# ska-telescope/ska-sdp-screen-fitting

Measured on AMD Instinct MI355X. Metric: screen-slots/sec (ant×time×freq) + FITS-cube wall-clock, KL 256² screen, higher is better.
Workload: dtype f64

## Files before the change

### include/screenfit.h

```cpp
#ifndef SCREENFIT_H
#define SCREENFIT_H

#include <stddef.h>
#include <stdint.h>

#ifdef __cplusplus
extern "C" {
#endif

#define SF_OK 0
#define SF_EINVAL (-22)
#define SF_ENOMEM (-12)
#define SF_EIO (-5)
#define SF_ENODEV (-19)

#define SF_MAX_DIR 60
#define SF_MAX_FIT_DIR 128
#define SF_MAX_EVAL_DIR 128

#define SF_SCREEN_PHASE 0
#define SF_SCREEN_TEC 1
#define SF_SCREEN_AMPLITUDE 2

#define SF_EVAL_NAN_SCRUB 1u
// ... 32 lines not shown
#define SF_OPT_EVAL_XCD_MAP 7
#define SF_OPT_EVAL_GROUPS 8
#define SF_OPT_EVAL_BANDS 9
#define SF_OPT_FIT_LEAN 10
#define SF_OPT_TESS_SLOTS 11
#define SF_OPT_TESS_WAVES 12
#define SF_OPT_TESS_TILE 13
#define SF_OPT_TESS_BOX 14
#define SF_OPT_EVAL_INT 15
#define SF_OPT_EVAL_WG_WAVES 16
#define SF_OPT_FIT_EIG_WAVES 17
#define SF_OPT_FIT_SUBSET_DELETION 18
#define SF_OPT_FIT_WIDE_CACHE 19
#define SF_OPT_FIT_WIDE_POOL_MB 20
#define SF_OPT_FIT_WIDE_POOL_MAX 21
#define SF_EVAL_KERNEL_AUTO 0
#define SF_EVAL_KERNEL_TILE 1
#define SF_EVAL_KERNEL_LDS4 2
#define SF_EVAL_KERNEL_LDS8 3
#define SF_EVAL_KERNEL_LDS16 4
#define SF_EVAL_KERNEL_LDS8H 5
#define SF_EVAL_KERNEL_LDS16H 6
#define SF_EVAL_KERNEL_TILE3 7
#define SF_EVAL_KERNEL_SHB 8
#define SF_EVAL_KERNEL_WIDE 9
int sf_get_eval_kernel(sf_ctx* ctx, int gain, unsigned flags, int* kernel);
#define SF_EVAL_CONTRACTION_F64 0
#define SF_EVAL_CONTRACTION_I8_DIGITS 1
int sf_get_eval_contraction(sf_ctx* ctx, int gain, unsigned flags, int* contraction);
int sf_set_option(sf_ctx* ctx, int option, int value);
// ... 6 lines not shown
                 double beta);
int sf_set_basis_wide(sf_ctx* ctx, const double* pp_host, int D, double r0,
                      double beta);
int sf_get_basis(sf_ctx* ctx, double* c_host, double* pinv_c_host,
                 double* u_host, double* eig_host);

int sf_set_piercepoints(sf_ctx* ctx, const double* pp_host, int D, double r0,
                        double beta);

int sf_kl_fit(sf_ctx* ctx, const double* phase, const float* weight, int T,
              int F, int A, const int* station_order_host,
              const sf_fit_params* params, double* coef, double* resid,
              float* w_out, int32_t* order_out);

int sf_get_fit_stats(sf_ctx* ctx, int* n_masks, int* n_general);

int sf_get_fit_pool(sf_ctx* ctx, uint64_t* masks_host, double* entries_host,
                    int max_masks, int* n_masks);
int sf_get_fit_pool_wide(sf_ctx* ctx, uint64_t* masks_host, double* entries_host,
                         int max_masks, int* n_masks);

int sf_set_grid(sf_ctx* ctx, const double* x_host, int nx,
                const double* y_host, int ny);

int sf_kl_eval(sf_ctx* ctx, const double* coef, int64_t S, float* out,
               int64_t ring_slots, unsigned flags);

int sf_kl_eval_gain(sf_ctx* ctx, const double* coef_phase,
                    const double* coef_xx, const double* coef_yy, int64_t S,
                    float* out, int64_t ring_slots, unsigned flags);
// ... 27 lines not shown
```

### ska-sdp-screen-fitting_amd/csrc/capi.hip

```cpp
#include <hip/hip_runtime.h>

#include <cmath>
#include <cstring>
#include <string>
#include <vector>

#include "sf_internal.h"

namespace sf {
static thread_local std::string g_last_error;
void set_error(const std::string& msg) { g_last_error = msg; }
}

using sf::set_error;

namespace {

int check_device(int device) {
  int n = 0;
  hipError_t e = hipGetDeviceCount(&n);
  if (e != hipSuccess || n == 0) {
    set_error("no HIP device available");
    return SF_ENODEV;
  }
// ... 104 lines not shown
  hipFree(ctx->d_pfrag);
  hipFree(ctx->d_cdig);
  hipFree(ctx->d_kdig);
  hipFree(ctx->d_kflag);
  if (ctx->kdig_read) (void)hipEventDestroy(ctx->kdig_read);
  hipFree(ctx->d_skip);
  hipFree(ctx->d_st_order);
  hipFree(ctx->d_keys);
  hipFree(ctx->d_ids);
  hipFree(ctx->d_pool_mask);
  hipFree(ctx->d_pool);
  hipFree(ctx->d_pool_status);
  hipFree(ctx->d_pos);
  hipFree(ctx->d_sigma);
  hipFree(ctx->d_class);
  hipFree(ctx->d_counters);
  hipFree(ctx->d_scratch);
  hipFree(ctx->d_wscratch);
  hipFree(ctx->d_oscratch);
  hipFree(ctx->d_gw);
  hipFree(ctx->d_smooth);
  hipFree(ctx->d_tess_tab);
  hipFree(ctx->d_trash);
  delete ctx;
  return SF_OK;
}

int sf_set_stream(sf_ctx* ctx, void* stream) {
  SF_REQUIRE(ctx, SF_EINVAL, "sf_set_stream: NULL context");
  ctx->stream = reinterpret_cast<hipStream_t>(stream);
// ... 43 lines not shown
  SF_REQUIRE(ctx, SF_EINVAL, "sf_set_option: NULL context");
  switch (option) {
    case SF_OPT_FIT_GENERAL:
      ctx->force_general = value != 0;
      return SF_OK;
    case SF_OPT_EVAL_KERNEL:
      SF_REQUIRE(value >= SF_EVAL_KERNEL_AUTO && value <= SF_EVAL_KERNEL_WIDE,
                 SF_EINVAL, "sf_set_option: unknown evaluation kernel");
      ctx->eval_kernel = value;
      return SF_OK;
    case SF_OPT_FIT_PACK:
      ctx->fit_pack = value != 0;
      return SF_OK;
    case SF_OPT_FIT_LEAN:
      ctx->fit_lean = value != 0;
      return SF_OK;
    case SF_OPT_EVAL_KS_PAD:
      SF_REQUIRE(value >= 0 && value <= 3, SF_EINVAL,
                 "sf_set_option: k-step padding must be 0..3");
      ctx->eval_ks_pad = value;
      return SF_OK;
    case SF_OPT_EVAL_SLEEP:
      SF_REQUIRE(value >= 0 && value <= 1000, SF_EINVAL,
                 "sf_set_option: eval sleep must be 0..1000");
      ctx->eval_sleep = value;
      return SF_OK;
    case SF_OPT_EVAL_XCD_MAP:
      SF_REQUIRE(value >= -1 && value <= 1, SF_EINVAL,
                 "sf_set_option: XCD map must be -1, 0 or 1");
      ctx->eval_xcd_map = value;
// ... 272 lines not shown
                        order_out);
}

int sf_get_fit_stats(sf_ctx* ctx, int* n_masks, int* n_general) {
  SF_REQUIRE(ctx, SF_EINVAL, "sf_get_fit_stats: NULL context");
  int c[4] = {0, 0, 0, 0};
  SF_HIP(hipSetDevice(ctx->device));
  SF_HIP(hipStreamSynchronize(ctx->stream));
  if (ctx->d_counters)
    SF_HIP(hipMemcpy(c, ctx->d_counters, sizeof(c), hipMemcpyDeviceToHost));
  if (n_masks) *n_masks = c[0];
  if (n_general) *n_general = c[2];
  return SF_OK;
}

int sf_get_fit_pool(sf_ctx* ctx, uint64_t* masks_host, double* entries_host,
                    int max_masks, int* n_masks) {
  SF_REQUIRE(ctx && n_masks && max_masks >= 0, SF_EINVAL, "sf_get_fit_pool: bad argument");
  SF_REQUIRE(max_masks == 0 || (masks_host && entries_host), SF_EINVAL,
             "sf_get_fit_pool: NULL output");
  SF_REQUIRE(!ctx->wide, SF_EINVAL,
             "sf_get_fit_pool: 64-bit mask keys; above SF_MAX_DIR directions "
             "(sf_set_basis_wide) call sf_get_fit_pool_wide");
  SF_HIP(hipSetDevice(ctx->device));
  SF_HIP(hipStreamSynchronize(ctx->stream));
  int c0 = 0;
  if (ctx->d_counters)
    SF_HIP(hipMemcpy(&c0, ctx->d_counters, sizeof(int), hipMemcpyDeviceToHost));
  const int n = ctx->pool_D == ctx->D && (size_t)c0 <= ctx->pool_cap ? c0 : 0;
  *n_masks = n;
// ... 315 lines not shown
```

### ska-sdp-screen-fitting_amd/csrc/kl_fit_fast.hip

```cpp
#include <hip/hip_runtime.h>

#include <algorithm>
#include <cmath>
#include <cstdlib>

#include "kl_fit_steps.h"
#include "sf_internal.h"

namespace sf {

constexpr size_t kLdsBytes = 160 * 1024;
constexpr double kTinyW = kPinvAtol * 1.001;
constexpr unsigned long long kEmptyKey = 0ull;

__device__ __forceinline__ unsigned long long mix64(unsigned long long x) {
  x ^= x >> 30;
  x *= 0xbf58476d1ce4e5b9ull;
  x ^= x >> 27;
  x *= 0x94d049bb133111ebull;
  x ^= x >> 31;
  return x;
}

__device__ int table_insert(unsigned long long* keys, int cap,
// ... 7 lines not shown
  }
  return -3;
}

__device__ int table_find(const unsigned long long* keys, int cap,
                          unsigned long long key) {
  int h = (int)(mix64(key) & (unsigned long long)(cap - 1));
  for (int probe = 0; probe < cap; ++probe) {
    const unsigned long long k = keys[h];
    if (k == key) return h;
    if (k == kEmptyKey) return -1;
    h = (h + 1) & (cap - 1);
  }
  return -1;
}

template <int GW>
__global__ __launch_bounds__(256) void kl_classify_kernel(
    const float* __restrict__ weight, int64_t S, int F, int A, int D,
    const int* __restrict__ st_order, const uint8_t* __restrict__ skip,
    int ref_skip, unsigned long long* __restrict__ keys, int cap,
    int* __restrict__ pos, uint8_t* __restrict__ cls,
    int* __restrict__ counters,
    double* __restrict__ coef, double* __restrict__ resid,
    float* __restrict__ w_out, int32_t* __restrict__ order_out) {
  constexpr int kPerWave = 64 / GW;
  const int l = lane();
  const int g = l / GW;
  const int d = l % GW;
  const int64_t s = ((int64_t)blockIdx.x * (blockDim.x / 64) + threadIdx.x / 64) *
// ... 599 lines not shown
    v0[l] = fabs(lm) > kPinvAtol ? sh / lm : 0.0;
  }
  lds_sync();
  double wa = 0.0;
  if (l < D)
#pragma unroll kMatVecUnroll
    for (int r = 0; r < D; ++r) wa += L.U[l * ld + r] * v0[r];
  lds_sync();
  white_d = wa;
  resid_d = phi_d - model_value<M>(screen_type, sall);
}

#ifndef SF_FIT_MINW
#define SF_FIT_MINW 4
#endif
template <bool SLOW, int SPW, bool LEAN>
__global__ __launch_bounds__(256, SLOW ? 1 : SF_FIT_MINW) void kl_fit_pass_kernel(
    int it, int niter, int64_t S, int F, int A, int D,
    const double* __restrict__ phase, const double* __restrict__ refph,
    int ref_sub, const double* __restrict__ g_u, const double* __restrict__ g_c,
    const double* __restrict__ g_eig, const int* __restrict__ st_order,
    const uint8_t* __restrict__ cls, int* __restrict__ pos,
    const int* __restrict__ ids, unsigned long long* __restrict__ keys, int cap,
    const double* __restrict__ pool, int pool_cap, int* __restrict__ counters,
    int screen_type, double nsigma, int adjust_order, double* __restrict__ coef,
    double* __restrict__ resid, float* __restrict__ w_out,
    int32_t* __restrict__ order_out) {
#pragma clang fp contract(off)
  extern __shared__ double smem[];
  const int ld = odd_ld(D);
  using G = Group<SPW>;
  using M = FitMath<!SLOW>;
  const G tm;
  constexpr bool CG = SPW == 1;
  const int nwaves = blockDim.x / 64;
  const int nslots = nwaves * SPW;
  const int wv = (threadIdx.x / 64) * SPW + G::index();
  const int d = G::lane();
  double* sU = smem;
  double* sC = CG ? nullptr : sU + D * ld;
  double* sl = sU + (CG ? 1 : 2) * D * ld;
  for (int e = threadIdx.x; e < D * D; e += blockDim.x) {
    const int r = e / D, c = e % D;
// ... 15 lines not shown
    L.pr = nullptr;
  } else {
    L.Vs = wb;
    L.G = wb + D * ld;
    L.M = L.G + D * ld;
    L.lams = (SLOW ? L.M + D * ld : L.G + D * ld);
    L.vec = L.lams + 64;
    L.cs = reinterpret_cast<double2*>(L.vec + 6 * 64);
    L.pr = reinterpret_cast<int2*>(L.cs + 64);
  }
  const uint8_t want = SLOW ? 2 : 0;

  for (int64_t s = (int64_t)blockIdx.x * nslots + wv; s < S;
       s += (int64_t)gridDim.x * nslots) {
    if (SLOW && cls[s] != want) continue;
    const uint8_t cl = SLOW ? want : cls[s];
    const int a = (int)(s % A);
    const int p0 = pos[s];
    const int64_t base = s * D;
    double phi_d = 0.0, w_d = 0.0, white_d = 0.0, resid_d = 0.0;
    if (d < D) {
      phi_d = phase_ref(phase, refph, ref_sub, s, a, A, D, d);
      w_d = (double)w_out[base + d];
      white_d = it == 0 ? 0.0 : coef[base + d];
      resid_d = it == 0 ? 0.0 : resid[base + d];
    }
    double order = (double)order_out[s];
    const double station_order = (double)st_order[a];
    if (cl != want) continue;
    int id = -1;
    if (p0 >= 0) {
      id = ids[p0];
      if (id < 0 || id >= pool_cap) {
        if (d == 0) atomicOr(counters + 3, 1);
        continue;
      }
    } else if (p0 == -3) {
      if (d == 0) atomicOr(counters + 3, 2);
      continue;
    }
    const bool unfl = (d < D) && (w_d > 0.0);
    const unsigned long long um = G::ballot(unfl);
    const int n_unfl = __popcll(um);

// ... 249 lines not shown
                       ctx->stream, ctx->d_c, D, ctx->d_pool_mask, (int)ctx->pool_cap, \
                       ctx->d_counters, ctx->d_pool, done);                            \
  } while (0)
    switch (nw) {
      case 1: SF_LAUNCH_EIG(1); break;
      case 2: SF_LAUNCH_EIG(2); break;
      case 4: SF_LAUNCH_EIG(4); break;
      default: SF_LAUNCH_EIG(3); break;
    }
#undef SF_LAUNCH_EIG
    SF_HIP(hipGetLastError());
  }
  return SF_OK;
}

template <bool SLOW, int SPW, bool LEAN>
static int launch_pass_spw(sf_ctx* ctx, int it, const sf_fit_params* p,
                           const RefSpec& r, int64_t S, int F, int A,
                           const double* phase, double* coef, double* resid,
                           float* w_out, int32_t* order_out) {
  const int D = ctx->D;
  const size_t shared = fast_shared_bytes(D, SPW == 1);
  const size_t slot = fast_wave_bytes(D, SLOW, LEAN);
  int nw = 1, best = 0;
  for (int k = 1; k <= 4; ++k) {
    const size_t per_wg = shared + (size_t)k * SPW * slot;
    if (per_wg > kLdsBytes) break;
    const int waves = k * (int)(kLdsBytes / per_wg);
    if (waves > best) {
      best = waves;
      nw = k;
    }
  }
  const size_t shm = shared + (size_t)nw * SPW * slot;
  if (shm > 64 * 1024)
    SF_HIP(hipFuncSetAttribute(
        reinterpret_cast<const void*>(&kl_fit_pass_kernel<SLOW, SPW, LEAN>),
        hipFuncAttributeMaxDynamicSharedMemorySize, (int)shm));
  int64_t blocks = (S + nw * SPW - 1) / (nw * SPW);
  if (blocks > 16384) blocks = 16384;
  hipLaunchKernelGGL((kl_fit_pass_kernel<SLOW, SPW, LEAN>), dim3((unsigned)blocks),
                     dim3(64 * nw), shm, ctx->stream, it, p->niter, S, F, A, D,
                     phase, r.refph, r.sub, ctx->d_u, ctx->d_c, ctx->d_eig,
                     ctx->d_st_order, ctx->d_class, ctx->d_pos, ctx->d_ids,
                     ctx->d_keys, (int)ctx->table_cap, ctx->d_pool,
                     (int)ctx->pool_cap, ctx->d_counters, p->screen_type,
                     p->nsigma, p->adjust_order, coef, resid, w_out, order_out);
  SF_HIP(hipGetLastError());
  return SF_OK;
}

template <bool SLOW>
static int launch_pass(sf_ctx* ctx, int it, const sf_fit_params* p,
                       const RefSpec& r, int64_t S, int F, int A,
                       const double* phase, double* coef, double* resid,
                       float* w_out, int32_t* order_out, bool lean) {
  const bool pack = !SLOW && ctx->D <= 32 && ctx->fit_pack;
  if (!SLOW && lean && ctx->fit_lean) {
    if (pack)
      return launch_pass_spw<false, 2, true>(ctx, it, p, r, S, F, A, phase, coef,
                                             resid, w_out, order_out);
    return launch_pass_spw<false, 1, true>(ctx, it, p, r, S, F, A, phase, coef,
                                           resid, w_out, order_out);
  }
  if (pack)
    return launch_pass_spw<SLOW, 2, false>(ctx, it, p, r, S, F, A, phase, coef,
                                           resid, w_out, order_out);
  return launch_pass_spw<SLOW, 1, false>(ctx, it, p, r, S, F, A, phase, coef, resid,
                                         w_out, order_out);
}

int launch_block_sigma(sf_ctx* ctx, int T, int F, int A, const double* phase,
                       const RefSpec& r, int screen_type, const double* resid,
                       const float* w_out) {
  hipLaunchKernelGGL(kl_block_sigma_kernel, dim3(F * A), dim3(256), 0,
                     ctx->stream, T, F, A, ctx->D, phase, r.refph, r.sub,
                     ctx->d_skip, r.skip, screen_type, resid, w_out,
                     ctx->d_sigma);
  SF_HIP(hipGetLastError());
  return SF_OK;
}

int fit_buffers(sf_ctx* ctx, int64_t S, int F, int A, double** resid,
                float** w_out, int32_t** order_out) {
// ... 6 lines not shown
    SF_TRY_RC(grow(&ctx->d_wscratch, ctx->wscratch_cap, n));
    *w_out = ctx->d_wscratch;
  }
  if (!*order_out) {
    SF_TRY_RC(grow(&ctx->d_oscratch, ctx->oscratch_cap, (size_t)S));
    *order_out = ctx->d_oscratch;
  }
  SF_TRY_RC(grow(&ctx->d_sigma, ctx->sigma_cap, (size_t)F * A));
  SF_TRY_RC(grow(&ctx->d_counters, ctx->counters_cap, 8));
  return SF_OK;
}

int launch_fit(sf_ctx* ctx, const double* phase, const float* weight, int T,
               int F, int A, const sf_fit_params* p, double* coef,
               double* resid, float* w_out, int32_t* order_out) {
  if (ctx->wide)
    return launch_fit_wide(ctx, phase, weight, T, F, A, p, coef, resid, w_out,
                           order_out);
  const int D = ctx->D;
  const int64_t S = (int64_t)T * F * A;
  const RefSpec r = ref_spec(p, A);
  SF_TRY_RC(launch_skip(ctx, phase, weight, T, F, A, r));

  static const char* env = std::getenv("SCREENFIT_FIT");
  if (ctx->force_general || (env && env[0] == 'g')) {
    if (p->screen_type == SF_SCREEN_AMPLITUDE ||
        (p->niter > 1 && p->screen_type != SF_SCREEN_PHASE)) {
      set_error("the general fit kernel handles phase (any niter) and tec (niter 1) only");
      return SF_EINVAL;
    }
// ... 37 lines not shown
  hipLaunchKernelGGL(kl_classify_kernel<W>, grid, dim3(256), 0, ctx->stream,    \
                     weight, S, F, A, D, ctx->d_st_order, ctx->d_skip, r.skip,  \
                     ctx->d_keys, cap, ctx->d_pos, ctx->d_class,               \
                     ctx->d_counters, coef, resid, w_out, order_out)
    switch (gw) {
      case 8: SF_CLASSIFY(8); break;
      case 16: SF_CLASSIFY(16); break;
      case 32: SF_CLASSIFY(32); break;
      default: SF_CLASSIFY(64); break;
    }
#undef SF_CLASSIFY
    SF_HIP(hipGetLastError());
  }

  const bool block_flags = p->screen_type != SF_SCREEN_PHASE;
  for (int it = 0; it < p->niter; ++it) {
    int n_slow = 0, n_nonuniform = 0;
    SF_TRY_RC(number_and_decompose(ctx, &n_slow, &n_nonuniform));
    SF_TRY_RC(launch_pass<false>(ctx, it, p, r, S, F, A, phase, coef, resid,
                               w_out, order_out, n_nonuniform == 0));
    if (n_slow > 0)
      SF_TRY_RC(launch_pass<true>(ctx, it, p, r, S, F, A, phase, coef, resid,
                                w_out, order_out, false));
    if (block_flags && it + 1 < p->niter) {
      SF_TRY_RC(launch_block_sigma(ctx, T, F, A, phase, r, p->screen_type, resid,
                                 w_out));
      hipLaunchKernelGGL(kl_block_flag_kernel, dim3((unsigned)((S + 255) / 256)),
                         dim3(256), 0, ctx->stream, S, F, A, D, phase, r.refph,
                         r.sub, ctx->d_class, p->screen_type, p->nsigma,
                         ctx->d_sigma, resid, w_out, ctx->d_keys, cap,
                         ctx->d_pos);
      SF_HIP(hipGetLastError());
    }
  }
  int err = 0;
  SF_HIP(hipMemcpyAsync(&err, ctx->d_counters + 3, sizeof(int),
                        hipMemcpyDeviceToHost, ctx->stream));
  SF_HIP(hipStreamSynchronize(ctx->stream));
  SF_REQUIRE((err & 3) == 0, SF_EIO, "sf_kl_fit: internal mask table overflow");
  SF_REQUIRE((err & 4) == 0, SF_EIO,
             "sf_kl_fit: lean fit pass saw non-uniform weights in a slot "
             "classified uniform (slot left unwritten)");
  SF_REQUIRE((err & 8) == 0, SF_EIO,
             "sf_kl_fit: a mask with every direction unflagged entered the "
             "subset-basis pool (its basis is the global one; left unbuilt)");
  return SF_OK;
}

}
```

### ska-sdp-screen-fitting_amd/csrc/kl_fit_steps.h

```cpp
#pragma once

#include <hip/hip_runtime.h>

#include <cmath>

#include "screenfit.h"
#include "sf_wave.h"

namespace sf {

constexpr double kPinvAtol = 1e-3;
constexpr int kJacobiMaxSweeps = 40;

__host__ __device__ inline int odd_ld(int n) { return n | 1; }

inline __device__ __noinline__ void nl_sincos(double x, double* s, double* c) { sincos(x, s, c); }
inline __device__ __noinline__ double nl_atan2(double y, double x) { return atan2(y, x); }
inline __device__ __noinline__ double nl_log10(double x) { return log10(x); }
inline __device__ __noinline__ double nl_pow(double x, double y) { return pow(x, y); }
inline __device__ __noinline__ double nl_log(double x) { return log(x); }
inline __device__ __noinline__ double nl_fmod(double x, double y) { return fmod(x, y); }

template <bool NI>
struct FitMath {
// ... 11 lines not shown
  }
  static __device__ __forceinline__ double ln(double x) {
    if constexpr (NI) return nl_log(x); else return log(x);
  }
  static __device__ __forceinline__ double mod(double x, double y) {
    if constexpr (NI) return nl_fmod(x, y); else return fmod(x, y);
  }
};

__device__ __forceinline__ double phase_ref(const double* phase,
                                            const double* refph, int sub,
                                            int64_t s, int a, int A, int D,
                                            int d) {
  double v = phase[s * D + d];
  if (refph) v -= refph[(s / A) * D + d];
  else if (sub >= 0) v -= phase[(s + (sub - a)) * D + d];
  return v;
}

template <class Math = FitMath<false>>
__device__ __forceinline__ double model_value(int screen_type, double x) {
  return screen_type == SF_SCREEN_AMPLITUDE ? Math::power(10.0, x) : x;
}

template <class Math = FitMath<false>>
__device__ __forceinline__ double screen_diff(int screen_type, double val,
                                              double resid) {
  if (screen_type == SF_SCREEN_AMPLITUDE)
    return Math::lg10(val) - Math::lg10(fabs(val - resid));
  return resid;
// ... 151 lines not shown
```

### ska-sdp-screen-fitting_amd/csrc/sf_internal.h

```cpp
#pragma once

#include <hip/hip_runtime.h>

#include <cstdint>
#include <string>

#include "screenfit.h"

namespace sf {

void set_error(const std::string& msg);

#define SF_HIP(call)                                                        \
  do {                                                                      \
    hipError_t e_ = (call);                                                 \
    if (e_ != hipSuccess) {                                                 \
      ::sf::set_error(std::string(#call) + ": " + hipGetErrorString(e_));   \
      return SF_EIO;                                                        \
    }                                                                       \
  } while (0)

#define SF_REQUIRE(cond, code, msg) \
  do {                              \
    if (!(cond)) {                  \
// ... 125 lines not shown
  size_t tess_tab_cap = 0;
  int force_general = 0;
  int eval_kernel = SF_EVAL_KERNEL_AUTO;
  int64_t eval_max_blocks = 0;
  int eval_ks_pad = 0;
  int eval_sleep = 0;
  int eval_xcd_map = -1;
  int eval_groups = 0;
  int eval_bands = 0;
  int tess_slots = 0;
  int tess_waves = 0;
  int tess_tile = 0;
  int tess_box = -1;
  int fit_pack = 1;
  int fit_lean = 1;
};

namespace sf {
constexpr int kEvalMaxKS = 15;
constexpr int kEvalWideMaxKS = SF_MAX_EVAL_DIR / 4;
inline bool eval_int_applies(const sf_ctx* ctx, bool gain, unsigned flags,
                             bool out_aligned16) {
  return !gain && ctx->dig_ok && ctx->d_cdig && ctx->eval_int != 0 &&
         (flags & SF_EVAL_FAST_SINCOS) && ctx->n_pix % 4 == 0 && out_aligned16 &&
         ctx->ksteps >= 12 && ctx->ksteps <= kEvalMaxKS;
}

struct RefSpec {
  int sub = -1;
  const double* refph = nullptr;
// ... 56 lines not shown
```

### ska-sdp-screen-fitting_amd/ska_sdp_screen_fitting_amd/_lib.py

```python

import contextlib
import ctypes
import os
import threading

import numpy as np

_HERE = os.path.dirname(os.path.abspath(__file__))
LIB_PATH = os.environ.get("SCREENFIT_LIB", os.path.join(_HERE, "libscreenfit.so"))

SF_SCREEN_PHASE = 0
SF_SCREEN_TEC = 1
SF_SCREEN_AMPLITUDE = 2
SF_EVAL_NAN_SCRUB = 1
SF_EVAL_FAST_SINCOS = 1 << 8
SF_EVAL_NT_STORES = 1 << 9
SF_EVAL_BIG_ENDIAN = 1 << 10
SF_MAX_DIR = 60
SF_MAX_FIT_DIR = 128
SF_MAX_EVAL_DIR = 128
SF_MAX_POINTS = 4096
SF_OPT_FIT_GENERAL = 1
SF_OPT_EVAL_KERNEL = 2
SF_OPT_EVAL_MAX_BLOCKS = 3
# ... 3 lines not shown
SF_OPT_EVAL_XCD_MAP = 7
SF_OPT_EVAL_GROUPS = 8
SF_OPT_EVAL_BANDS = 9
SF_OPT_FIT_LEAN = 10
SF_OPT_TESS_SLOTS = 11
SF_OPT_TESS_WAVES = 12
SF_OPT_TESS_TILE = 13
SF_OPT_TESS_BOX = 14
SF_OPT_EVAL_INT = 15
SF_OPT_EVAL_WG_WAVES = 16
SF_OPT_FIT_EIG_WAVES = 17
SF_OPT_FIT_SUBSET_DELETION = 18
SF_OPT_FIT_WIDE_CACHE = 19
SF_OPT_FIT_WIDE_POOL_MB = 20
SF_OPT_FIT_WIDE_POOL_MAX = 21
SF_EVAL_KERNEL_AUTO = 0
SF_EVAL_KERNEL_TILE = 1
SF_EVAL_KERNEL_LDS4 = 2
SF_EVAL_KERNEL_LDS8 = 3
SF_EVAL_KERNEL_LDS16 = 4
SF_EVAL_KERNEL_LDS8H = 5
SF_EVAL_KERNEL_LDS16H = 6
SF_EVAL_KERNEL_TILE3 = 7
SF_EVAL_KERNEL_SHB = 8
SF_EVAL_KERNEL_WIDE = 9
EVAL_KERNEL_NAMES = {SF_EVAL_KERNEL_TILE: "kl_eval_kernel",
                     SF_EVAL_KERNEL_LDS4: "kl_eval_lds_kernel<4 waves>",
                     SF_EVAL_KERNEL_LDS8: "kl_eval_lds_kernel<8 waves>",
                     SF_EVAL_KERNEL_LDS16: "kl_eval_lds_kernel<16 waves>",
                     SF_EVAL_KERNEL_LDS8H: "kl_eval_lds_kernel<8 waves, 2 tiles>",
                     SF_EVAL_KERNEL_LDS16H: "kl_eval_lds_kernel<16 waves, 2 tiles>",
                     SF_EVAL_KERNEL_TILE3: "kl_eval_kernel<3 waves/SIMD>",
                     SF_EVAL_KERNEL_SHB: "kl_eval_kernel<Cpix in LDS>",
                     SF_EVAL_KERNEL_WIDE: "kl_eval_wide_kernel"}

EXPORTED = (
    "sf_version", "sf_last_error", "sf_create", "sf_destroy", "sf_set_stream",
    "sf_synchronize", "sf_set_option", "sf_get_eval_kernel", "sf_get_eval_contraction", "sf_alloc", "sf_free", "sf_copy_h2d", "sf_copy_d2h",
    "sf_set_basis", "sf_set_basis_wide", "sf_set_piercepoints", "sf_get_basis", "sf_kl_fit", "sf_get_fit_stats", "sf_get_fit_pool",
    "sf_get_fit_pool_wide",
    "sf_stream_create", "sf_stream_destroy", "sf_device_cus",
    "sf_set_grid", "sf_kl_eval", "sf_kl_eval_gain", "sf_kl_eval_sums",
    "sf_tess_fill", "sf_smooth",
    "sf_set_points", "sf_kl_eval_points", "sf_kl_eval_point_values",
    "sf_kl_eval_values",
)


_identity = {}


def library_identity(path=None):
    import hashlib
    p = os.path.realpath(path or LIB_PATH)
# ... 45 lines not shown
            "sf_synchronize": ([vp], c_int),
            "sf_set_option": ([vp, c_int, c_int], c_int),
            "sf_get_eval_kernel": ([vp, c_int, ctypes.c_uint, ip], c_int),
            "sf_get_eval_contraction": ([vp, c_int, ctypes.c_uint, ip], c_int),
            "sf_alloc": ([vp, ctypes.c_size_t, ctypes.POINTER(vp)], c_int),
            "sf_free": ([vp, vp], c_int),
            "sf_copy_h2d": ([vp, vp, vp, ctypes.c_size_t], c_int),
            "sf_copy_d2h": ([vp, vp, vp, ctypes.c_size_t], c_int),
            "sf_set_basis": ([vp, vp, c_int, c_dbl, c_dbl], c_int),
            "sf_set_basis_wide": ([vp, vp, c_int, c_dbl, c_dbl], c_int),
            "sf_set_piercepoints": ([vp, vp, c_int, c_dbl, c_dbl], c_int),
            "sf_get_basis": ([vp, vp, vp, vp, vp], c_int),
            "sf_kl_fit": ([vp, vp, vp, c_int, c_int, c_int, ip,
                           ctypes.POINTER(FitParams), vp, vp, vp, vp], c_int),
            "sf_get_fit_stats": ([vp, ip, ip], c_int),
            "sf_get_fit_pool": ([vp, vp, vp, c_int, ip], c_int),
            "sf_get_fit_pool_wide": ([vp, vp, vp, c_int, ip], c_int),
            "sf_set_grid": ([vp, vp, c_int, vp, c_int], c_int),
            "sf_kl_eval": ([vp, vp, i64, vp, i64, ctypes.c_uint], c_int),
            "sf_stream_create": ([vp, ctypes.POINTER(c_int), c_int,
                                  ctypes.POINTER(vp)], c_int),
            "sf_stream_destroy": ([vp, vp], c_int),
            "sf_device_cus": ([vp, ctypes.POINTER(c_int)], c_int),
            "sf_kl_eval_gain": ([vp, vp, vp, vp, i64, vp, i64, ctypes.c_uint],
                                c_int),
            "sf_kl_eval_sums": ([vp, vp, vp, vp, i64, vp, i64, ctypes.c_uint, vp],
                                c_int),
            "sf_tess_fill": ([vp, vp, c_int, c_int, vp, vp, vp, c_int, i64, vp,
                              i64, c_dbl, ctypes.c_uint], c_int),
            "sf_smooth": ([vp, vp, c_int, c_int, i64, c_dbl, ctypes.c_uint], c_int),
# ... 151 lines not shown
            self.h, self._dev(phase, np.float64, n, "phase"),
            self._dev(weight, np.float32, n, "weight"), int(T), int(F), int(A),
            so.ctypes.data_as(ctypes.POINTER(ctypes.c_int)),
            ctypes.byref(prm), self._dev(coef, np.float64, n, "coef"),
            self._dev(resid, np.float64, n, "resid"),
            self._dev(w_out, np.float32, n, "w_out"),
            self._dev(order_out, np.int32, n // max(self.D, 1), "order_out")),
            "sf_kl_fit")

    def fit_stats(self):
        nm, ng = ctypes.c_int(), ctypes.c_int()
        _check(self.lib.sf_get_fit_stats(self.h, ctypes.byref(nm), ctypes.byref(ng)),
               "sf_get_fit_stats")
        return {"n_masks": nm.value, "n_general": ng.value}

    def fit_pool(self):
        n = ctypes.c_int(0)
        _check(self.lib.sf_get_fit_pool(self.h, None, None, 0, ctypes.byref(n)),
               "sf_get_fit_pool")
        D = self.D
        masks = np.zeros(n.value, np.uint64)
        ent = np.zeros((n.value, D * D + D))
        if n.value:
            _check(self.lib.sf_get_fit_pool(self.h, masks.ctypes.data, ent.ctypes.data,
                                            n.value, ctypes.byref(n)), "sf_get_fit_pool")
        order = np.argsort(masks, kind="stable")
        masks, ent = masks[order], ent[order]
        for k, m in enumerate(masks):
            n = bin(int(m)).count("1")
            u = ent[k, :D * D].reshape(D, D)
# ... 173 lines not shown
```

Baseline: 6.309 million.

## Add dense one-slot-per-lane fit kernel for uniform-weight first iteration

Adds a dense KL fit kernel in which each lane of a 64-wide block fits one slot entirely in registers, using a padded basis and its transpose precomputed on device. It runs on the first iteration when every slot is fast-class and uniform. Slots that finish are marked final, and slots with outliers or order changes are handed to the existing lean pass kernel, which now skips slots it does not own. The goal is to avoid per-slot mask-table lookups and wave-cooperative overhead for the common case. The cost is an extra launch, heavy register use for larger direction counts, and a second code path whose results must agree with the existing fit.

```diff
diff --git a/include/screenfit.h b/include/screenfit.h
--- a/include/screenfit.h
+++ b/include/screenfit.h
@@ -70,6 +70,8 @@
 #define SF_OPT_FIT_WIDE_CACHE 19
 #define SF_OPT_FIT_WIDE_POOL_MB 20
 #define SF_OPT_FIT_WIDE_POOL_MAX 21
+#define SF_OPT_FIT_DENSE 22
+#define SF_FIT_DENSE_MAX_DIR 24
 #define SF_EVAL_KERNEL_AUTO 0
 #define SF_EVAL_KERNEL_TILE 1
 #define SF_EVAL_KERNEL_LDS4 2
@@ -106,6 +108,8 @@
               float* w_out, int32_t* order_out);
 
 int sf_get_fit_stats(sf_ctx* ctx, int* n_masks, int* n_general);
+
+int sf_get_fit_dense_stats(sf_ctx* ctx, int64_t* n_dense, int64_t* n_handed_over);
 
 int sf_get_fit_pool(sf_ctx* ctx, uint64_t* masks_host, double* entries_host,
                     int max_masks, int* n_masks);
diff --git a/ska-sdp-screen-fitting_amd/csrc/capi.hip b/ska-sdp-screen-fitting_amd/csrc/capi.hip
--- a/ska-sdp-screen-fitting_amd/csrc/capi.hip
+++ b/ska-sdp-screen-fitting_amd/csrc/capi.hip
@@ -142,6 +142,7 @@
   hipFree(ctx->d_pos);
   hipFree(ctx->d_sigma);
   hipFree(ctx->d_class);
+  hipFree(ctx->d_dense_basis);
   hipFree(ctx->d_counters);
   hipFree(ctx->d_scratch);
   hipFree(ctx->d_wscratch);
@@ -215,6 +216,11 @@
       return SF_OK;
     case SF_OPT_FIT_LEAN:
       ctx->fit_lean = value != 0;
+      return SF_OK;
+    case SF_OPT_FIT_DENSE:
+      SF_REQUIRE(value == 0 || value == 1, SF_EINVAL,
+                 "sf_set_option: fit dense must be 0 or 1");
+      ctx->fit_dense = value;
       return SF_OK;
     case SF_OPT_EVAL_KS_PAD:
       SF_REQUIRE(value >= 0 && value <= 3, SF_EINVAL,
@@ -517,6 +523,13 @@
   return SF_OK;
 }
 
+int sf_get_fit_dense_stats(sf_ctx* ctx, int64_t* n_dense, int64_t* n_handed_over) {
+  SF_REQUIRE(ctx, SF_EINVAL, "sf_get_fit_dense_stats: NULL context");
+  if (n_dense) *n_dense = ctx->fit_n_dense;
+  if (n_handed_over) *n_handed_over = ctx->fit_n_handed;
+  return SF_OK;
+}
+
 int sf_get_fit_pool(sf_ctx* ctx, uint64_t* masks_host, double* entries_host,
                     int max_masks, int* n_masks) {
   SF_REQUIRE(ctx && n_masks && max_masks >= 0, SF_EINVAL, "sf_get_fit_pool: bad argument");
diff --git a/ska-sdp-screen-fitting_amd/csrc/kl_fit_dense.h b/ska-sdp-screen-fitting_amd/csrc/kl_fit_dense.h
--- /dev/null
+++ b/ska-sdp-screen-fitting_amd/csrc/kl_fit_dense.h
@@ -0,0 +1,297 @@
+#pragma once
+
+namespace sf {
+
+constexpr uint8_t kClsDenseFinal = 3;
+constexpr uint8_t kClsDenseHanded = 4;
+
+__device__ __forceinline__ bool pass_owns(uint8_t cl, int it) {
+  return cl == 0 || (cl == kClsDenseHanded && it > 0);
+}
+
+constexpr int kDenseMaxD = SF_FIT_DENSE_MAX_DIR;
+static_assert(kDenseMaxD == 24, "launch_fit_dense: bounds 4, 8, ... 24");
+constexpr int kDenseMinD = 3;
+inline int dense_bound(int D) { return D <= 4 ? 4 : (D + 3) / 4 * 4; }
+inline size_t dense_basis_doubles(int DB) { return (size_t)2 * DB * DB + DB; }
+
+__global__ __launch_bounds__(256) void kl_dense_basis_kernel(
+    const double* __restrict__ g_u, const double* __restrict__ g_eig, int D,
+    int DB, double* __restrict__ out) {
+  const int n = 2 * DB * DB + DB;
+  for (int e = threadIdx.x; e < n; e += blockDim.x) {
+    double v = 0.0;
+    if (e < 2 * DB * DB) {
+      const bool tr = e >= DB * DB;
+      const int q = tr ? e - DB * DB : e;
+      const int r = q / DB, c = q % DB;
+      if (r < D && c < D) v = tr ? g_u[c * D + r] : g_u[r * D + c];
+    } else if (e - 2 * DB * DB < D) {
+      v = g_eig[e - 2 * DB * DB];
+    }
+    out[e] = v;
+  }
+}
+
+inline __device__ __noinline__ double2 nl_sincos2(double x) {
+  double s, c;
+  sincos(x, &s, &c);
+  return make_double2(s, c);
+}
+
+template <int DB>
+__device__ __forceinline__ double half_wave_sum(const double (&x)[DB]) {
+#pragma clang fp contract(off)
+  double y[32];
+#pragma unroll
+  for (int i = 0; i < 32; ++i) y[i] = i < DB ? x[i < DB ? i : 0] : 0.0;
+#pragma unroll
+  for (int o = 16; o > 0; o >>= 1) {
+#pragma unroll
+    for (int i = 0; i < o; ++i) y[i] = y[i] + y[i + o];
+  }
+  return y[0];
+}
+
+template <int DB>
+__global__ __launch_bounds__(64, 2) void kl_fit_dense_kernel(
+    int niter, int64_t S, int A, int D, const double* __restrict__ phase,
+    const double* __restrict__ refph, int ref_sub,
+    const double* __restrict__ basis, const int* __restrict__ st_order,
+    uint8_t* __restrict__ cls, int* __restrict__ pos,
+    unsigned long long* __restrict__ keys, int cap, int* __restrict__ counters,
+    double nsigma, int adjust_order, double* __restrict__ coef,
+    double* __restrict__ resid, float* __restrict__ w_out,
+    int32_t* __restrict__ order_out) {
+#pragma clang fp contract(off)
+  static_assert(DB < 32, "half_wave_sum: a slot is half a wave");
+  using M = FitMath<true>;
+  constexpr int kPitch = DB | 1;
+  __shared__ double sP[64 * kPitch];
+  __shared__ double sQ[64 * kPitch];
+  __shared__ int64_t sTf[64];
+  __shared__ int sAnt[64];
+  const int l = lane();
+  const int64_t s0 = (int64_t)blockIdx.x * 64;
+  const int64_t s = s0 + l;
+  const bool take = s < S && cls[s] == 0 && pos[s] == -1;
+  const unsigned long long taken = __ballot(take);
+  if (taken == 0ull) return;
+
+  const int64_t tf = s / A;
+  const int a = (int)(s - tf * A);
+  sTf[l] = tf;
+  sAnt[l] = a;
+  lds_sync();
+  const int64_t rest = (S - s0) * D;
+  const int e_end = rest < 64 * D ? (int)rest : 64 * D;
+  const int step_j = 64 / D, step_d = 64 - step_j * D;
+  {
+    int j = l / D, d = l - j * D;
+    for (int e = l; e < e_end; e += 64) {
+      sP[j * kPitch + d] =
+          phase_ref_at(phase, refph, ref_sub, s0 + j, sTf[j], sAnt[j], D, d);
+      j += step_j;
+      d += step_d;
+      if (d >= D) {
+        d -= D;
+        ++j;
+      }
+    }
+  }
+  lds_sync();
+
+  double* P = sP + l * kPitch;
+  double* Q = sQ + l * kPitch;
+  const double* U = basis;
+  const double* UT = basis + DB * DB;
+  const double* lam = basis + 2 * DB * DB;
+  double wu = 0.0, order = 0.0, station_order = 0.0;
+  if (take) {
+    wu = (double)w_out[s * D];
+    station_order = (double)st_order[a];
+    order = (double)order_out[s];
+    if (order > D - 1) order = D - 1;
+    const int K = (int)order;
+
+    double a1[DB], a2[DB];
+#pragma unroll
+    for (int i = 0; i < DB; ++i) a1[i] = a2[i] = 0.0;
+    for (int p = 0; p < D; ++p) {
+      const double2 sc = nl_sincos2(P[p]);
+      const double rc = wu * sc.y;
+      const double rs = wu * sc.x;
+      const double* u = U + p * DB;
+#pragma unroll
+      for (int i = 0; i < DB; ++i) {
+        a1[i] += u[i] * rc;
+        a2[i] += u[i] * rs;
+      }
+    }
+#pragma unroll
+    for (int i = 0; i < DB; ++i) {
+      if (i < K) {
+        const bool keep = fabs(lam[i]) > kPinvAtol;
+        a1[i] = keep ? a1[i] / wu : 0.0;
+        a2[i] = keep ? a2[i] / wu : 0.0;
+      }
+    }
+    double cre[DB], cim[DB];
+#pragma unroll
+    for (int i = 0; i < DB; ++i) {
+      cre[i] = cim[i] = 0.0;
+      Q[i] = a1[i];
+    }
+    for (int k = 0; k < D - 1; ++k) {
+      if (k < K) {
+        const double x = Q[k];
+        const double* u = UT + k * DB;
+#pragma unroll
+        for (int i = 0; i < DB; ++i) cre[i] += u[i] * x;
+      }
+    }
+#pragma unroll
+    for (int i = 0; i < DB; ++i) Q[i] = a2[i];
+    for (int k = 0; k < D - 1; ++k) {
+      if (k < K) {
+        const double x = Q[k];
+        const double* u = UT + k * DB;
+#pragma unroll
+        for (int i = 0; i < DB; ++i) cim[i] += u[i] * x;
+      }
+    }
+#pragma unroll
+    for (int i = 0; i < DB; ++i)
+      if (i < D) Q[i] = M::arctan2(cim[i], cre[i]);
+    double sh[DB];
+#pragma unroll
+    for (int i = 0; i < DB; ++i) sh[i] = 0.0;
+    for (int p = 0; p < D; ++p) {
+      const double x = Q[p];
+      const double* u = U + p * DB;
+#pragma unroll
+      for (int i = 0; i < DB; ++i) sh[i] += u[i] * x;
+    }
+    double white[DB], cw[DB];
+#pragma unroll
+    for (int i = 0; i < DB; ++i) {
+      white[i] = cw[i] = 0.0;
+      const double lm = lam[i];
+      Q[i] = fabs(lm) > kPinvAtol ? sh[i] / lm : 0.0;
+    }
+    for (int r = 0; r < D; ++r) {
+      const double x = Q[r];
+      const double* u = UT + r * DB;
+#pragma unroll
+      for (int i = 0; i < DB; ++i) white[i] += u[i] * x;
+    }
+#pragma unroll
+    for (int i = 0; i < DB; ++i) Q[i] = fabs(lam[i]) > kPinvAtol ? sh[i] : 0.0;
+    for (int r = 0; r < D; ++r) {
+      const double x = Q[r];
+      const double* u = UT + r * DB;
+#pragma unroll
+      for (int i = 0; i < DB; ++i) cw[i] += u[i] * x;
+    }
+#pragma unroll
+    for (int i = 0; i < DB; ++i) {
+      if (i < D) {
+        P[i] = P[i] - model_value<M>(SF_SCREEN_PHASE, cw[i]);
+        Q[i] = white[i];
+      }
+    }
+  }
+  lds_sync();
+  {
+    int j = l / D, d = l - j * D;
+    for (int e = l; e < e_end; e += 64) {
+      if ((taken >> j) & 1ull) {
+        coef[s0 * D + e] = sQ[j * kPitch + d];
+        resid[s0 * D + e] = sP[j * kPitch + d];
+      }
+      j += step_j;
+      d += step_d;
+      if (d >= D) {
+        d -= D;
+        ++j;
+      }
+    }
+  }
+  lds_sync();
+
+  bool fin = false;
+  if (take) {
+    fin = true;
+    if (niter > 1) {
+      double sn[DB], cn[DB], one[DB];
+      unsigned inc = 0u;
+#pragma unroll
+      for (int i = 0; i < DB; ++i) {
+        sn[i] = cn[i] = 0.0;
+        if (i < D) {
+          double r = M::mod(P[i], 2.0 * M_PI);
+          if (r < -M_PI) r += 2.0 * M_PI;
+          if (r > M_PI) r -= 2.0 * M_PI;
+          Q[i] = r;
+          if ((wu != 0.0) && !isnan(r)) {
+            const double2 sc = nl_sincos2(r);
+            sn[i] = sc.x;
+            cn[i] = sc.y;
+            inc |= 1u << i;
+          }
+        }
+      }
+#pragma unroll
+      for (int i = 0; i < DB; ++i) one[i] = ((inc >> i) & 1u) ? 1.0 : 0.0;
+      const double t0 = half_wave_sum(one);
+      const double t1 = half_wave_sum(sn);
+      const double t2 = half_wave_sum(cn);
+      const double ms = t1 / t0;
+      const double mc = t2 / t0;
+      const double stdv = sqrt(-2.0 * M::ln(hypot(ms, mc)));
+      unsigned outl = 0u;
+#pragma unroll
+      for (int i = 0; i < DB; ++i)
+        if (i < D && fabs(Q[i]) > nsigma * stdv) outl |= 1u << i;
+      if (outl != 0u) {
+        fin = false;
+        for (int i = 0; i < D; ++i)
+          if ((outl >> i) & 1u) w_out[s * D + i] = 0.0f;
+        const unsigned long long nm =
+            ((1ull << D) - 1ull) & ~(unsigned long long)outl;
+        pos[s] = (nm == 0ull) ? -2 : table_insert(keys, cap, nm);
+      } else if (adjust_order) {
+        double q0[DB], q1[DB], q2[DB];
+#pragma unroll
+        for (int i = 0; i < DB; ++i) {
+          q0[i] = q1[i] = q2[i] = 0.0;
+          if (i < D) {
+            const bool same = ((inc >> i) & 1u) && Q[i] == P[i];
+            const double2 sc = same ? make_double2(sn[i], cn[i]) : nl_sincos2(P[i]);
+            q0[i] = wu;
+            q1[i] = sc.x * sc.x * wu;
+            q2[i] = sc.y * sc.y * wu;
+          }
+        }
+        const double r0 = half_wave_sum(q0);
+        const double r1 = half_wave_sum(q1);
+        const double r2 = half_wave_sum(q2);
+        const double m1 = r1 / r0;
+        const double m2 = r2 / r0;
+        const double redchi2 = (1.0 - hypot(m1, m2)) * r0 / (D - order);
+        OrderWalk walk;
+        double moved = order;
+        fin = walk.template step<M>(0, redchi2, D, station_order, moved);
+      }
+    }
+    order_out[s] = (int32_t)order;
+    cls[s] = fin ? kClsDenseFinal : kClsDenseHanded;
+  }
+  const unsigned long long handed = __ballot(take && !fin);
+  if (l == 0) {
+    atomicAdd(counters + 6, __popcll(taken));
+    if (handed != 0ull) atomicAdd(counters + 7, __popcll(handed));
+  }
+}
+
+}
diff --git a/ska-sdp-screen-fitting_amd/csrc/kl_fit_fast.hip b/ska-sdp-screen-fitting_amd/csrc/kl_fit_fast.hip
--- a/ska-sdp-screen-fitting_amd/csrc/kl_fit_fast.hip
+++ b/ska-sdp-screen-fitting_amd/csrc/kl_fit_fast.hip
@@ -45,6 +45,12 @@
   }
   return -1;
 }
+
+}
+
+#include "kl_fit_dense.h"
+
+namespace sf {
 
 template <int GW>
 __global__ __launch_bounds__(256) void kl_classify_kernel(
@@ -674,7 +680,7 @@
 #ifndef SF_FIT_MINW
 #define SF_FIT_MINW 4
 #endif
-template <bool SLOW, int SPW, bool LEAN>
+template <bool SLOW, int SPW, bool LEAN, bool DENSE = false>
 __global__ __launch_bounds__(256, SLOW ? 1 : SF_FIT_MINW) void kl_fit_pass_kernel(
     int it, int niter, int64_t S, int F, int A, int D,
     const double* __restrict__ phase, const double* __restrict__ refph,
@@ -687,6 +693,7 @@
     double* __restrict__ resid, float* __restrict__ w_out,
     int32_t* __restrict__ order_out) {
 #pragma clang fp contract(off)
+  static_assert(!DENSE || (!SLOW && LEAN), "the dense kernel serves the lean fast class");
   extern __shared__ double smem[];
   const int ld = odd_ld(D);
   using G = Group<SPW>;
@@ -732,6 +739,7 @@
   for (int64_t s = (int64_t)blockIdx.x * nslots + wv; s < S;
        s += (int64_t)gridDim.x * nslots) {
     if (SLOW && cls[s] != want) continue;
+    if (DENSE && !pass_owns(cls[s], it)) continue;
     const uint8_t cl = SLOW ? want : cls[s];
     const int a = (int)(s % A);
     const int p0 = pos[s];
@@ -745,7 +753,7 @@
     }
     double order = (double)order_out[s];
     const double station_order = (double)st_order[a];
-    if (cl != want) continue;
+    if (DENSE ? !pass_owns(cl, it) : cl != want) continue;
     int id = -1;
     if (p0 >= 0) {
       id = ids[p0];
@@ -1025,7 +1033,7 @@
   return SF_OK;
 }
 
-template <bool SLOW, int SPW, bool LEAN>
+template <bool SLOW, int SPW, bool LEAN, bool DENSE = false>
 static int launch_pass_spw(sf_ctx* ctx, int it, const sf_fit_params* p,
                            const RefSpec& r, int64_t S, int F, int A,
                            const double* phase, double* coef, double* resid,
@@ -1046,11 +1054,11 @@
   const size_t shm = shared + (size_t)nw * SPW * slot;
   if (shm > 64 * 1024)
     SF_HIP(hipFuncSetAttribute(
-        reinterpret_cast<const void*>(&kl_fit_pass_kernel<SLOW, SPW, LEAN>),
+        reinterpret_cast<const void*>(&kl_fit_pass_kernel<SLOW, SPW, LEAN, DENSE>),
         hipFuncAttributeMaxDynamicSharedMemorySize, (int)shm));
   int64_t blocks = (S + nw * SPW - 1) / (nw * SPW);
   if (blocks > 16384) blocks = 16384;
-  hipLaunchKernelGGL((kl_fit_pass_kernel<SLOW, SPW, LEAN>), dim3((unsigned)blocks),
+  hipLaunchKernelGGL((kl_fit_pass_kernel<SLOW, SPW, LEAN, DENSE>), dim3((unsigned)blocks),
                      dim3(64 * nw), shm, ctx->stream, it, p->niter, S, F, A, D,
                      phase, r.refph, r.sub, ctx->d_u, ctx->d_c, ctx->d_eig,
                      ctx->d_st_order, ctx->d_class, ctx->d_pos, ctx->d_ids,
@@ -1065,9 +1073,17 @@
 static int launch_pass(sf_ctx* ctx, int it, const sf_fit_params* p,
                        const RefSpec& r, int64_t S, int F, int A,
                        const double* phase, double* coef, double* resid,
-                       float* w_out, int32_t* order_out, bool lean) {
+                       float* w_out, int32_t* order_out, bool lean,
+                       bool dense = false) {
   const bool pack = !SLOW && ctx->D <= 32 && ctx->fit_pack;
   if (!SLOW && lean && ctx->fit_lean) {
+    if (dense) {
+      if (pack)
+        return launch_pass_spw<false, 2, true, true>(ctx, it, p, r, S, F, A, phase,
+                                                     coef, resid, w_out, order_out);
+      return launch_pass_spw<false, 1, true, true>(ctx, it, p, r, S, F, A, phase,
+                                                   coef, resid, w_out, order_out);
+    }
     if (pack)
       return launch_pass_spw<false, 2, true>(ctx, it, p, r, S, F, A, phase, coef,
                                              resid, w_out, order_out);
@@ -1079,6 +1095,37 @@
                                            resid, w_out, order_out);
   return launch_pass_spw<SLOW, 1, false>(ctx, it, p, r, S, F, A, phase, coef, resid,
                                          w_out, order_out);
+}
+
+static int launch_fit_dense(sf_ctx* ctx, const sf_fit_params* p, const RefSpec& r,
+                            int64_t S, int A, const double* phase, double* coef,
+                            double* resid, float* w_out, int32_t* order_out) {
+  const int D = ctx->D;
+  const int DB = dense_bound(D);
+  SF_TRY_RC(grow(&ctx->d_dense_basis, ctx->dense_basis_cap,
+                 dense_basis_doubles(kDenseMaxD)));
+  hipLaunchKernelGGL(kl_dense_basis_kernel, dim3(1), dim3(256), 0, ctx->stream,
+                     ctx->d_u, ctx->d_eig, D, DB, ctx->d_dense_basis);
+  SF_HIP(hipGetLastError());
+  const dim3 grid((unsigned)((S + 63) / 64));
+#define SF_DENSE(B)                                                            \
+  hipLaunchKernelGGL(kl_fit_dense_kernel<B>, grid, dim3(64), 0, ctx->stream,   \
+                     p->niter, S, A, D, phase, r.refph, r.sub,                 \
+                     ctx->d_dense_basis, ctx->d_st_order, ctx->d_class,        \
+                     ctx->d_pos, ctx->d_keys, (int)ctx->table_cap,             \
+                     ctx->d_counters, p->nsigma, p->adjust_order, coef, resid, \
+                     w_out, order_out)
+  switch (DB) {
+    case 4: SF_DENSE(4); break;
+    case 8: SF_DENSE(8); break;
+    case 12: SF_DENSE(12); break;
+    case 16: SF_DENSE(16); break;
+    case 20: SF_DENSE(20); break;
+    default: SF_DENSE(24); break;
+  }
+#undef SF_DENSE
+  SF_HIP(hipGetLastError());
+  return SF_OK;
 }
 
 int launch_block_sigma(sf_ctx* ctx, int T, int F, int A, const double* phase,
@@ -1115,6 +1162,7 @@
 int launch_fit(sf_ctx* ctx, const double* phase, const float* weight, int T,
                int F, int A, const sf_fit_params* p, double* coef,
                double* resid, float* w_out, int32_t* order_out) {
+  ctx->fit_n_dense = ctx->fit_n_handed = 0;
   if (ctx->wide)
     return launch_fit_wide(ctx, phase, weight, T, F, A, p, coef, resid, w_out,
                            order_out);
@@ -1182,11 +1230,19 @@
   }
 
   const bool block_flags = p->screen_type != SF_SCREEN_PHASE;
+  const bool dense_ok = ctx->fit_dense && ctx->fit_lean && !block_flags &&
+                        D >= kDenseMinD && D <= kDenseMaxD;
+  bool dense = false;
   for (int it = 0; it < p->niter; ++it) {
     int n_slow = 0, n_nonuniform = 0;
     SF_TRY_RC(number_and_decompose(ctx, &n_slow, &n_nonuniform));
+    if (it == 0 && dense_ok && n_nonuniform == 0 && n_slow == 0) {
+      SF_TRY_RC(launch_fit_dense(ctx, p, r, S, A, phase, coef, resid, w_out,
+                                 order_out));
+      dense = true;
+    }
     SF_TRY_RC(launch_pass<false>(ctx, it, p, r, S, F, A, phase, coef, resid,
-                               w_out, order_out, n_nonuniform == 0));
+                               w_out, order_out, n_nonuniform == 0, dense));
     if (n_slow > 0)
       SF_TRY_RC(launch_pass<true>(ctx, it, p, r, S, F, A, phase, coef, resid,
                                 w_out, order_out, false));
@@ -1201,10 +1257,13 @@
       SF_HIP(hipGetLastError());
     }
   }
-  int err = 0;
-  SF_HIP(hipMemcpyAsync(&err, ctx->d_counters + 3, sizeof(int),
+  int tail[5] = {0, 0, 0, 0, 0};
+  SF_HIP(hipMemcpyAsync(tail, ctx->d_counters + 3, sizeof(tail),
                         hipMemcpyDeviceToHost, ctx->stream));
   SF_HIP(hipStreamSynchronize(ctx->stream));
+  const int err = tail[0];
+  ctx->fit_n_dense = tail[3];
+  ctx->fit_n_handed = tail[4];
   SF_REQUIRE((err & 3) == 0, SF_EIO, "sf_kl_fit: internal mask table overflow");
   SF_REQUIRE((err & 4) == 0, SF_EIO,
              "sf_kl_fit: lean fit pass saw non-uniform weights in a slot "
diff --git a/ska-sdp-screen-fitting_amd/csrc/kl_fit_steps.h b/ska-sdp-screen-fitting_amd/csrc/kl_fit_steps.h
--- a/ska-sdp-screen-fitting_amd/csrc/kl_fit_steps.h
+++ b/ska-sdp-screen-fitting_amd/csrc/kl_fit_steps.h
@@ -49,6 +49,15 @@
                                             int d) {
   double v = phase[s * D + d];
   if (refph) v -= refph[(s / A) * D + d];
+  else if (sub >= 0) v -= phase[(s + (sub - a)) * D + d];
+  return v;
+}
+__device__ __forceinline__ double phase_ref_at(const double* phase,
+                                               const double* refph, int sub,
+                                               int64_t s, int64_t tf, int a,
+                                               int D, int d) {
+  double v = phase[s * D + d];
+  if (refph) v -= refph[tf * D + d];
   else if (sub >= 0) v -= phase[(s + (sub - a)) * D + d];
   return v;
 }
diff --git a/ska-sdp-screen-fitting_amd/csrc/sf_internal.h b/ska-sdp-screen-fitting_amd/csrc/sf_internal.h
--- a/ska-sdp-screen-fitting_amd/csrc/sf_internal.h
+++ b/ska-sdp-screen-fitting_amd/csrc/sf_internal.h
@@ -163,6 +163,11 @@
   int tess_box = -1;
   int fit_pack = 1;
   int fit_lean = 1;
+  int fit_dense = 1;
+  double* d_dense_basis = nullptr;
+  size_t dense_basis_cap = 0;
+  int64_t fit_n_dense = 0;
+  int64_t fit_n_handed = 0;
 };
 
 namespace sf {
diff --git a/ska-sdp-screen-fitting_amd/ska_sdp_screen_fitting_amd/_lib.py b/ska-sdp-screen-fitting_amd/ska_sdp_screen_fitting_amd/_lib.py
--- a/ska-sdp-screen-fitting_amd/ska_sdp_screen_fitting_amd/_lib.py
+++ b/ska-sdp-screen-fitting_amd/ska_sdp_screen_fitting_amd/_lib.py
@@ -41,6 +41,8 @@
 SF_OPT_FIT_WIDE_CACHE = 19
 SF_OPT_FIT_WIDE_POOL_MB = 20
 SF_OPT_FIT_WIDE_POOL_MAX = 21
+SF_OPT_FIT_DENSE = 22
+SF_FIT_DENSE_MAX_DIR = 24
 SF_EVAL_KERNEL_AUTO = 0
 SF_EVAL_KERNEL_TILE = 1
 SF_EVAL_KERNEL_LDS4 = 2
@@ -64,7 +66,7 @@
 EXPORTED = (
     "sf_version", "sf_last_error", "sf_create", "sf_destroy", "sf_set_stream",
     "sf_synchronize", "sf_set_option", "sf_get_eval_kernel", "sf_get_eval_contraction", "sf_alloc", "sf_free", "sf_copy_h2d", "sf_copy_d2h",
-    "sf_set_basis", "sf_set_basis_wide", "sf_set_piercepoints", "sf_get_basis", "sf_kl_fit", "sf_get_fit_stats", "sf_get_fit_pool",
+    "sf_set_basis", "sf_set_basis_wide", "sf_set_piercepoints", "sf_get_basis", "sf_kl_fit", "sf_get_fit_stats", "sf_get_fit_dense_stats", "sf_get_fit_pool",
     "sf_get_fit_pool_wide",
     "sf_stream_create", "sf_stream_destroy", "sf_device_cus",
     "sf_set_grid", "sf_kl_eval", "sf_kl_eval_gain", "sf_kl_eval_sums",
@@ -140,6 +142,8 @@
             "sf_kl_fit": ([vp, vp, vp, c_int, c_int, c_int, ip,
                            ctypes.POINTER(FitParams), vp, vp, vp, vp], c_int),
             "sf_get_fit_stats": ([vp, ip, ip], c_int),
+            "sf_get_fit_dense_stats": ([vp, ctypes.POINTER(i64),
+                                        ctypes.POINTER(i64)], c_int),
             "sf_get_fit_pool": ([vp, vp, vp, c_int, ip], c_int),
             "sf_get_fit_pool_wide": ([vp, vp, vp, c_int, ip], c_int),
             "sf_set_grid": ([vp, vp, c_int, vp, c_int], c_int),
@@ -321,6 +325,13 @@
                "sf_get_fit_stats")
         return {"n_masks": nm.value, "n_general": ng.value}
 
+    def fit_dense_stats(self):
+        nd, nh = ctypes.c_int64(), ctypes.c_int64()
+        _check(self.lib.sf_get_fit_dense_stats(self.h, ctypes.byref(nd),
+                                               ctypes.byref(nh)),
+               "sf_get_fit_dense_stats")
+        return {"n_dense": nd.value, "n_handed_over": nh.value}
+
     def fit_pool(self):
         n = ctypes.c_int(0)
         _check(self.lib.sf_get_fit_pool(self.h, None, None, 0, ctypes.byref(n)),
```

Result: no change. 6.341 million, median of 6 (+0.5%).
